# SrinivasBaskar1995/DistributedVolunteerComputing

Hardware: AMD Instinct MI355X
Metric: samples/sec GPT-2-small local-SGD (higher is better)
Workload: dtype bf16; 1 GPU; model=gpt2, global_batch=64, per_peer_batch=64, seq_len=1024, parallelism=local-sgd dp1 H=4 allreduce=direct

## Files before the change

distributedvolunteercomputing_amd/config.py:

```python
from __future__ import annotations

import contextlib
import dataclasses
import os
import threading


def _bool(s: str) -> bool:
    return s.strip().lower() in ("1", "true", "yes", "on")


@dataclasses.dataclass
class RuntimeConfig:
    gemm: str = "lib"
    mlp: str = "fused"
    narrow_gemm: str = "lib"
    mlp_grad_fwd: bool = True
    gemm_fwd: str = "lib"
    dgrad_ps: bool = True
    gemm_wgrad: str = "vcx"
    wgrad_wide: bool = True
    wgrad_ragged: bool = False
    gemm_select: bool = False
    wgrad_big_split_min_m: int = 16384
    async_wgrad: bool = False
    lmhead_chunk: int = 0
    force_reference_ops: bool = False
    tunableop: str = "on"
    tunableop_file: str = ""
    offload_arch: str = "gfx950"
    colour_native: bool = True
    register_source: bool = True
# ... 13 lines not shown
    elastic_liveness: bool = True
    elastic_stage_joins: str = "gloo"
    uplink_pipeline: str = "relay"
    shared_source_root: str = ""
    store_port_train: int = 29611
    store_port_video: int = 29612
    trace_dir: str = ""
    metrics_dir: str = ""


_ENV = {
    "gemm": ("VCX_GEMM", str),
    "mlp": ("VCX_MLP", str),
    "dgrad_ps": ("VCX_DGRAD_PS", _bool),
    "mlp_grad_fwd": ("VCX_MLP_GRAD_FWD", _bool),
    "narrow_gemm": ("VCX_NARROW_GEMM", str),
    "resnet_conv1x1": ("VCX_RESNET_CONV1X1", str),
    "resnet_bn": ("VCX_RESNET_BN", str),
    "resnet_join": ("VCX_RESNET_JOIN", _bool),
    "engine_batch": ("VCX_ENGINE_BATCH", int),
    "conv3x3_wgrad": ("VCX_CONV3X3_WGRAD", str),
    "conv3x3_fwd": ("VCX_CONV3X3_FWD", str),
    "resnet_proj_join": ("VCX_RESNET_PROJ_JOIN", _bool),
    "bn_layer_ws": ("VCX_BN_LAYER_WS", _bool),
    "conv_find": ("VCX_CONV_FIND", _bool),
    "gemm_wgrad": ("VCX_GEMM_WGRAD", str),
    "gemm_fwd": ("VCX_GEMM_FWD", str),
    "wgrad_wide": ("VCX_WGRAD_WIDE", _bool),
    "wgrad_ragged": ("VCX_WGRAD_RAGGED", _bool),
    "gemm_select": ("VCX_GEMM_SELECT", _bool),
# ... 83 lines not shown
```

distributedvolunteercomputing_amd/csrc/bindings.cpp:

```cpp
#include <torch/extension.h>
#include <map>
#include <mutex>
#include <thread>
#include <tuple>
#include <c10/hip/HIPStream.h>
#include <hip/hip_runtime.h>

#include "kernels/vcx_api.h"

namespace {

hipStream_t cur_stream() { return c10::hip::getCurrentHIPStream().stream(); }

#define CHECK_CUDA(x) TORCH_CHECK((x).is_cuda(), #x " must be a GPU tensor")
#define CHECK_CONTIG(x) TORCH_CHECK((x).is_contiguous(), #x " must be contiguous")
#define CHECK_DT(x, dt) TORCH_CHECK((x).scalar_type() == (dt), #x " has wrong dtype ", (x).scalar_type())
#define CHECK_IN(x, dt) \
  CHECK_CUDA(x);        \
  CHECK_CONTIG(x);      \
  CHECK_DT(x, dt)

const auto kBF = at::kBFloat16;
const auto kF = at::kFloat;

// ... 487 lines not shown
              "x under 2 GB");
  for (const at::Tensor* t : {&dy, &x, &out})
    TORCH_CHECK(reinterpret_cast<uintptr_t>(t->data_ptr()) % 16 == 0, "gemm_wg_conv3x3: 16-B aligned base pointers");
  at::Tensor ws = at::empty({splits, Cout, 9 * Cin}, dy.options().dtype(at::kFloat));
  vcx_gemm_wg_conv3x3(dy.data_ptr(), x.data_ptr(), ws.data_ptr<float>(), out.data_ptr(), (int)Cout, (int)Cin, (int)imgs,
                      (int)H, (int)W, (int)stride, (int)splits, accumulate ? 1 : 0, cur_stream());
}

at::Tensor transpose_bf16(at::Tensor src, c10::optional<at::Tensor> dst) {
  TORCH_CHECK(src.is_cuda() && src.dim() == 2 && src.is_contiguous() && src.scalar_type() == at::kBFloat16,
              "transpose_bf16: contiguous 2-D bf16");
  at::Tensor out = dst ? *dst : at::empty({src.size(1), src.size(0)}, src.options());
  TORCH_CHECK(out.size(0) == src.size(1) && out.size(1) == src.size(0) && out.is_contiguous(), "transpose_bf16: dst");
  vcx_transpose_bf16(src.data_ptr(), out.data_ptr(), (int)src.size(0), (int)src.size(1), cur_stream());
  return out;
}

void add_f32_into_bf16(at::Tensor in, at::Tensor out, bool accumulate, bool zero_in) {
  TORCH_CHECK(in.is_cuda() && in.scalar_type() == at::kFloat && out.scalar_type() == at::kBFloat16 &&
                  in.numel() == out.numel() && in.is_contiguous() && out.is_contiguous() &&
                  in.get_device() == out.get_device() && in.numel() < (int64_t(1) << 31),
              "add_f32_into_bf16: fp32 in, bf16 out of equal size on one device");
  vcx_add_f32_into_bf16(in.data_ptr<float>(), out.data_ptr(), (int)in.numel(), accumulate ? 1 : 0, zero_in ? 1 : 0,
                        cur_stream());
}

void reduce_bcast_bf16(at::Tensor in, c10::optional<at::Tensor> out, c10::optional<at::Tensor> mine, int64_t P) {
  TORCH_CHECK(in.is_cuda() && in.scalar_type() == at::kBFloat16 && in.is_contiguous(), "reduce_bcast: bf16 cuda in");
  const int64_t n = in.numel() / P;
  TORCH_CHECK(P > 0 && n * P == in.numel() && n % 8 == 0, "reduce_bcast: numel must be P * n with n % 8 == 0");
// ... 503 lines not shown
  m.def("gemm_f_conv3x3", &gemm_f_conv3x3, py::arg("x"), py::arg("w"), py::arg("out"), py::arg("stride"),
        py::arg("bias") = py::none(), py::arg("waves") = 0, py::arg("splits") = -1, py::arg("flip_taps") = false);
  m.def("gemm_f_splits", &gemm_f_splits, py::arg("M"), py::arg("N"), py::arg("K"));
  m.def("gemm_f", &gemm_f, py::arg("a"), py::arg("b"), py::arg("out"), py::arg("bias") = py::none(),
        py::arg("waves") = 0, py::arg("splits") = -1);
  m.def("gemm_wg_supported", &gemm_wg_supported, py::arg("M"), py::arg("N"), py::arg("K"), py::arg("splits") = 0);
  m.def("gemm_wg_conv3x3_supported", &gemm_wg_conv3x3_supported, py::arg("Cout"), py::arg("Cin"), py::arg("imgs"),
        py::arg("H"), py::arg("W"), py::arg("stride"));
  m.def("gemm_wg_conv3x3", &gemm_wg_conv3x3, py::arg("dy"), py::arg("x"), py::arg("out"), py::arg("accumulate") = false,
        py::arg("stride") = 1, py::arg("splits") = 0);
  m.def("gemm_wg", &gemm_wg, py::arg("a"), py::arg("b"), py::arg("out"), py::arg("accumulate") = false,
        py::arg("splits") = 0, py::arg("loaders") = 8);
  m.def("gemm_nt", &gemm_nt, py::arg("a"), py::arg("b"), py::arg("c"), py::arg("c2") = py::none(),
        py::arg("bias") = py::none(), py::arg("colsum") = py::none(), py::arg("epi") = 0);
  m.def("transpose_bf16", &transpose_bf16, py::arg("src"), py::arg("dst") = py::none());
  m.def("subsample_nhwc", &subsample_nhwc, py::arg("x"), py::arg("stride"));
  m.def("subsample_add_nhwc", &subsample_add_nhwc, py::arg("full"), py::arg("g"), py::arg("stride"));
  m.def("bcast_hw_nhwc", &bcast_hw_nhwc, py::arg("g"), py::arg("H"), py::arg("W"), py::arg("scale"));
  m.def("add_f32_into_bf16", &add_f32_into_bf16, py::arg("src"), py::arg("out"), py::arg("accumulate"),
        py::arg("zero_src") = false);
  m.def("splitk_reduce", &splitk_reduce);
  m.def("ln_fwd", &ln_fwd);
  m.def("ln_bwd", &ln_bwd, pybind11::arg("dy"), pybind11::arg("x"), pybind11::arg("w"), pybind11::arg("mean"),
        pybind11::arg("rstd"), pybind11::arg("dres"), pybind11::arg("has_bias"), pybind11::arg("rms"),
        pybind11::arg("has_bb"), pybind11::arg("dw_out") = pybind11::none(), pybind11::arg("db_out") = pybind11::none(),
        pybind11::arg("dbb_out") = pybind11::none());
  m.def("colsum_bf16", &colsum_bf16, pybind11::arg("y"), pybind11::arg("out") = pybind11::none());
  m.def("gelu_fwd", &gelu_fwd);
  m.def("bias_gelu_fwd", &bias_gelu_fwd);
  m.def("bias_gelu_bwd", &bias_gelu_bwd, pybind11::arg("x"), pybind11::arg("b"), pybind11::arg("dy"),
// ... 27 lines not shown
```

distributedvolunteercomputing_amd/csrc/kernels/gemm.hip:

```cpp
#include <type_traits>

#include "lds_ring.h"

namespace vcx {
namespace gemm {

constexpr int BM = 256, BN = 256, BKS = 32, NSLOT = 4, NT = 512;
constexpr int ROWB = BKS * 2;
constexpr int SLOT_A = BM * ROWB;
constexpr int SLOT_BYTES = (BM + BN) * ROWB;
constexpr int LDS_BYTES = NSLOT * SLOT_BYTES;

enum Epi { EPI_STORE = 0, EPI_BIAS = 1, EPI_BIAS_GELU = 2, EPI_DGELU = 3, EPI_BIAS_RELU = 4 };

__device__ __forceinline__ void glds16(const bf16* g, char* lds) {
  __builtin_amdgcn_global_load_lds((const __attribute__((address_space(1))) void*)g,
                                   (__attribute__((address_space(3))) void*)lds, 16, 0, 0);
}

__device__ __forceinline__ float gelu_tanh(float x) {
  const float u2 = 1.5957691216057308f * fmaf(0.044715f * x, x * x, x);
  return x / (1.f + __expf(-u2));
}

// ... 211 lines not shown
  if constexpr (EPI == EPI_DGELU) {
#pragma unroll
    for (int j = 0; j < 4; ++j)
#pragma unroll
      for (int t = 0; t < 4; ++t) {
        float v = cs[j][t];
        v += __shfl_xor(v, 1, 64);
        v += __shfl_xor(v, 2, 64);
        v += __shfl_xor(v, 4, 64);
        v += __shfl_xor(v, 8, 64);
        if ((lane & 15) == 0) atomicAdd(colsum + ncol + 16 * j + t, v);
      }
  }
}

__global__ void __launch_bounds__(256) transpose_bf16_kernel(const bf16* __restrict__ src, bf16* __restrict__ dst,
                                                             int R, int Cc) {
  __shared__ bf16 t[64][65];
  const int r0 = blockIdx.y * 64, c0 = blockIdx.x * 64;
  for (int e = threadIdx.x; e < 64 * 64; e += 256) {
    const int rr = e >> 6, cc = e & 63;
    if (r0 + rr < R && c0 + cc < Cc) t[rr][cc] = src[(int64_t)(r0 + rr) * Cc + c0 + cc];
  }
  __syncthreads();
  for (int e = threadIdx.x; e < 64 * 64; e += 256) {
    const int cc = e >> 6, rr = e & 63;
    if (r0 + rr < R && c0 + cc < Cc) dst[(int64_t)(c0 + cc) * R + r0 + rr] = t[rr][cc];
  }
}

__global__ void __launch_bounds__(256) transpose_bf16_v8_kernel(const bf16* __restrict__ src, bf16* __restrict__ dst,
                                                                int R, int Cc) {
  __shared__ __attribute__((aligned(16))) bf16 t[64][72];
  const int r0 = blockIdx.y * 64, c0 = blockIdx.x * 64;
#pragma unroll
  for (int i = 0; i < 2; ++i) {
    const int e = threadIdx.x + 256 * i, rr = e >> 3, cc = (e & 7) * 8;
    if (r0 + rr < R && c0 + cc < Cc) *(bf16x8*)&t[rr][cc] = *(const bf16x8*)(src + (int64_t)(r0 + rr) * Cc + c0 + cc);
  }
  __syncthreads();
#pragma unroll
  for (int i = 0; i < 2; ++i) {
    const int e = threadIdx.x + 256 * i, cc = e >> 3, rr = (e & 7) * 8;
    if (c0 + cc < Cc && r0 + rr < R) {
      bf16x8 v;
#pragma unroll
      for (int j = 0; j < 8; ++j) v[j] = t[rr + j][cc];
      *(bf16x8*)(dst + (int64_t)(c0 + cc) * R + r0 + rr) = v;
    }
  }
}

__global__ void __launch_bounds__(256) add_f32_into_bf16_kernel(float* __restrict__ in, bf16* __restrict__ out, int n,
                                                                int accumulate, int zero_in) {
  const int i = blockIdx.x * 256 + threadIdx.x;
  if (i < n) {
    out[i] = (bf16)((accumulate ? (float)out[i] : 0.f) + in[i]);
    if (zero_in) in[i] = 0.f;
  }
}

}
}

using namespace vcx;
// ... 31 lines not shown
    case EPI_BIAS_RELU: args(gemm_nt_kernel<EPI_BIAS_RELU>); break;
    default: args(gemm_nt_kernel<EPI_DGELU>); break;
  }
}

void vcx_transpose_bf16(const void* src, void* dst, int R, int Cc, hipStream_t s) {
  if (R % 8 == 0 && Cc % 8 == 0 && ((uintptr_t)src | (uintptr_t)dst) % 16 == 0) {
    hipLaunchKernelGGL(gemm::transpose_bf16_v8_kernel, dim3((Cc + 63) / 64, (R + 63) / 64), dim3(256), 0, s,
                       (const bf16*)src, (bf16*)dst, R, Cc);
    return;
  }
  hipLaunchKernelGGL(gemm::transpose_bf16_kernel, dim3((Cc + 63) / 64, (R + 63) / 64), dim3(256), 0, s,
                     (const bf16*)src, (bf16*)dst, R, Cc);
}

void vcx_add_f32_into_bf16(float* in, void* out, int n, int accumulate, int zero_in, hipStream_t s) {
  hipLaunchKernelGGL(gemm::add_f32_into_bf16_kernel, dim3((n + 255) / 256), dim3(256), 0, s, in, (bf16*)out, n,
                     accumulate, zero_in);
}
```

distributedvolunteercomputing_amd/csrc/kernels/vcx_api.h:

```cpp
#pragma once
#include <hip/hip_runtime.h>
#include <stdint.h>

void vcx_grad_sumsq(const void* g, int64_t n, float* ostate, hipStream_t s);
void vcx_adam_prologue(float* ostate, float max_norm, hipStream_t s);
void vcx_adamw_flat(void* param, const void* grad, float* master, float* m, float* v, int64_t n, int64_t n_decay,
                    const float* ostate, float beta1, float beta2, float eps, float wd, hipStream_t s);
void vcx_adamw_flat_compact(void* param, const void* grad, float* master, uint8_t* m_code, uint8_t* m_exp,
                            void* v_half, uint8_t* v_exp, int64_t n, int64_t n_decay, const float* ostate,
                            double beta1, double beta2, float eps, float wd, hipStream_t s);
void vcx_optstate_encode(const float* m, const float* v, uint8_t* m_code, uint8_t* m_exp, void* v_half,
                         uint8_t* v_exp, int64_t n, hipStream_t s);
void vcx_optstate_decode(const uint8_t* m_code, const uint8_t* m_exp, const void* v_half, const uint8_t* v_exp,
                         float* m, float* v, int64_t n, hipStream_t s);
void vcx_lsgd_delta(const float* master, const float* anchor, void* delta, int64_t n, hipStream_t s);
void vcx_lsgd_apply(const void* avg, float* anchor, float* master, void* param, float* mom, int64_t n,
                    float outer_lr, float mu, int nesterov, float avg_scale, hipStream_t s);
void vcx_f32_to_bf16(const float* src, void* dst, int64_t n, hipStream_t s);
void vcx_axpy_bf16(const void* src, void* acc, int64_t n, float scale, hipStream_t s);
bool vcx_gemm_wg_supported(int M, int N, int K, int splits);
int vcx_gemm_wg_splits(int M, int N, int K);
void vcx_gemm_wg(const void* A, const void* B, float* Cpart, void* out, int M, int N, int K, int lda, int ldb,
                 int splits, int accumulate, int loaders, hipStream_t s);
bool vcx_gemm_wg_conv3x3_supported(int Cout, int Cin, int tokens, int64_t xbytes, int splits);
// ... 5 lines not shown
void vcx_gemm_f(const void* A, const void* B, void* C, const void* bias, int M, int N, int K, int lda, int ldb,
                int ldc, int waves, int splits, float* ws, hipStream_t s);
bool vcx_gemm_f_conv3x3_supported(int imgs, int H, int W, int Cin, int Cout, int stride);
void vcx_gemm_f_conv3x3(const void* x, const void* w, void* y, const void* bias, int imgs, int H, int W, int Cin,
                        int Cout, int stride, int waves, int splits, float* ws, int flip, int tap_major,
                        hipStream_t s);
bool vcx_gemm_nt_supported(int M, int N, int K);
bool vcx_gemm_nt_supported_epi(int M, int N, int K, int epi);
void vcx_gemm_nt(const void* A, const void* B, void* C, void* C2, const void* bias, float* colsum, int M, int N, int K,
                 int lda, int ldb, int ldc, int epi, hipStream_t s);
bool vcx_gemm_ps_supported(int M, int N, int K, int epi);
int vcx_gemm_ps_grid(int M, int N, int grid_cap);
void vcx_gemm_ps(const void* A, const void* B, void* C, void* C2, const void* bias, float* colsum, int M, int N,
                 int K, int lda, int ldb, int ldc, int epi, int grid_cap, hipStream_t s);
void vcx_transpose_bf16(const void* src, void* dst, int R, int Cc, hipStream_t s);
void vcx_add_f32_into_bf16(float* in, void* out, int n, int accumulate, int zero_in, hipStream_t s);
void vcx_reduce_bcast_bf16(const void* in, void* out, void* mine, int P, int64_t n, hipStream_t s);
void vcx_splitk_reduce(const void* part, void* acc, int S, int64_t n, int accumulate, hipStream_t s);

void vcx_trimmed_reduce_bcast_bf16(const void* in, void* out, void* mine, int P, int64_t n, int trim,
                                   uint32_t live_mask, float inv, int64_t* counts, hipStream_t s);
void vcx_cclip_reduce_bcast_bf16(const void* in, void* out, void* mine, int P, int64_t n, uint32_t live_mask, float tau,
                                 int iters, float* weights, float* workspace, hipStream_t s);
int64_t vcx_cclip_workspace_floats(int P, int64_t n);
int vcx_cclip_max_workgroups();

void vcx_ln_fwd(const void* a, const void* b, void* xout, void* y, const void* w, const void* bias, float* mean,
                float* rstd, int R, int C, float eps, int rms, const void* bb, hipStream_t s);
int vcx_bias_gelu_partials(int R);
void vcx_bias_gelu_fwd(const void* x, const void* b, void* y, int R, int F, hipStream_t s);
// ... 58 lines not shown
```

distributedvolunteercomputing_amd/models/gpt2.py:

```python
from __future__ import annotations

import math
from dataclasses import dataclass

import torch
import torch.nn as nn
import torch.nn.functional as F
from torch.nn.attention import SDPBackend, sdpa_kernel

from .. import ops

_SDPA_BACKENDS = [SDPBackend.EFFICIENT_ATTENTION, SDPBackend.FLASH_ATTENTION, SDPBackend.MATH]


@dataclass
class GPT2Config:
    vocab_size: int = 50257
    padded_vocab: int = 50304
    n_ctx: int = 1024
    n_layer: int = 12
    n_head: int = 12
    n_embd: int = 768
    ln_eps: float = 1e-5

    @staticmethod
# ... 15 lines not shown
        C = cfg.n_embd
        self.n_head = cfg.n_head
        self.ln1_w = nn.Parameter(torch.ones(C))
        self.ln1_b = nn.Parameter(torch.zeros(C))
        self.attn_w = nn.Parameter(torch.empty(3 * C, C))
        self.attn_b = nn.Parameter(torch.zeros(3 * C))
        self.proj_w = nn.Parameter(torch.empty(C, C))
        self.proj_b = nn.Parameter(torch.zeros(C))
        self.ln2_w = nn.Parameter(torch.ones(C))
        self.ln2_b = nn.Parameter(torch.zeros(C))
        self.fc_w = nn.Parameter(torch.empty(4 * C, C))
        self.fc_b = nn.Parameter(torch.zeros(4 * C))
        self.fc2_w = nn.Parameter(torch.empty(C, 4 * C))
        self.fc2_b = nn.Parameter(torch.zeros(C))

    def attn(self, h):
        B, T, C = h.shape
        H = self.n_head
        fuse = (C // H == 64 and h.dtype == torch.bfloat16 and ops.native_linear_ok(self.attn_w)
                and self.attn_b.requires_grad)
        qkv = ops.linear(h, self.attn_w, self.attn_b, bias_grad_elsewhere=fuse).view(B, T, 3, H, C // H)
        if C // H == 64 and qkv.is_cuda:
            y = ops.causal_attention(qkv, bias=self.attn_b if fuse else None)
        else:
            q, k, v = qkv.permute(2, 0, 3, 1, 4).unbind(0)
            with sdpa_kernel(_SDPA_BACKENDS):
                y = F.scaled_dot_product_attention(q, k, v, is_causal=True)
            y = y.transpose(1, 2)
        return ops.linear(y.reshape(B, T, C), self.proj_w)

    def mlp(self, h):
        return ops.mlp_gelu(h, self.fc_w, self.fc_b, self.fc2_w)


class GPT2(nn.Module):
    def __init__(self, cfg: GPT2Config):
        super().__init__()
        self.cfg = cfg
        C = cfg.n_embd
        self.wte = nn.Parameter(torch.empty(cfg.padded_vocab, C))
        self.wpe = nn.Parameter(torch.empty(cfg.n_ctx, C))
        self.blocks = nn.ModuleList([Block(cfg) for _ in range(cfg.n_layer)])
        self.lnf_w = nn.Parameter(torch.ones(C))
        self.lnf_b = nn.Parameter(torch.zeros(C))
        self.reset_parameters()

    @torch.no_grad()
    def reset_parameters(self, seed: int | None = None):
        g = torch.Generator(device="cpu")
        g.manual_seed(1234 if seed is None else seed)
        std = 0.02
        proj_std = 0.02 / math.sqrt(2 * self.cfg.n_layer)

        def init(p, s):
            p.copy_(torch.randn(p.shape, generator=g) * s)

        init(self.wte, std)
        init(self.wpe, 0.01)
        for b in self.blocks:
# ... 1 lines not shown
            init(b.proj_w, proj_std)
            init(b.fc_w, std)
            init(b.fc2_w, proj_std)

    def num_params(self, non_embedding=True):
        n = sum(p.numel() for p in self.parameters())
        if non_embedding:
            n -= self.wpe.numel()
        return n

    def flops_per_token(self, T: int) -> float:
        c = self.cfg
        N = self.num_params(non_embedding=True)
        return 6.0 * N + 12.0 * c.n_layer * c.n_embd * T

    def forward(self, idx, targets=None):
        B, T = idx.shape
        cfg = self.cfg
        x = ops.embed(idx, self.wte, self.wpe)
        eps = cfg.ln_eps
        blocks = self.blocks
        h, resid = ops.add_layernorm(x, None, blocks[0].ln1_w, blocks[0].ln1_b, eps)
        for i, blk in enumerate(blocks):
            a = blk.attn(h)
            h, resid = ops.add_layernorm(resid, a, blk.ln2_w, blk.ln2_b, eps, branch_bias=blk.proj_b)
            m = blk.mlp(h)
            if i + 1 < len(blocks):
                nxt = blocks[i + 1]
                h, resid = ops.add_layernorm(resid, m, nxt.ln1_w, nxt.ln1_b, eps, branch_bias=blk.fc2_b)
            else:
                h, resid = ops.add_layernorm(resid, m, self.lnf_w, self.lnf_b, eps, branch_bias=blk.fc2_b)
        if targets is None:
            return ops.linear(h, self.wte)[..., : cfg.vocab_size]
        return ops.lm_head_cross_entropy(h, self.wte, targets, cfg.vocab_size)
```

distributedvolunteercomputing_amd/ops/__init__.py:

```python
from ._lib import available as native_available, native
from .activations import bias_gelu, gelu, swiglu
from .attention import causal_attention, fused_bias_grad_ok, gqa_attention
from .embedding import embed
from .linear import gemm_nt, linear, mlp_gelu, native_linear_ok, set_gemm_backend, wgrad
from .loss import cross_entropy, lm_head_cross_entropy
from .norm import add_layernorm, add_rmsnorm, layernorm, rmsnorm
from .rope import rope_qkv
from .optim import (CompactState, adamw_flat_compact, adamw_step, adamw_step_compact, axpy_bf16,
                    check_compact_betas, f32_to_bf16, lsgd_apply, lsgd_delta, new_ostate, reduce_bcast_bf16)
from .robust import (centered_clip_reference, cclip_reduce_bcast_bf16, trimmed_mean_reference,
                     trimmed_reduce_bcast_bf16)
```

distributedvolunteercomputing_amd/ops/linear.py:

```python
from __future__ import annotations

import torch
import torch.nn.functional as F


from .. import config
from ._lib import grad_buffer, native, use_native

MIN_ROWS_PER_SPLIT = 2048


def set_gemm_backend(name: str):
    config.update(gemm="lib" if name == "lib" else "vcx")


def gemm_nt_ok(M: int, N: int, K: int, t) -> bool:
    return (config.get().gemm == "vcx" and use_native(t) and t.dtype == torch.bfloat16
            and bool(native().gemm_nt_supported(M, N, K)))


def gemm_nt(a, b, bias=None, out=None):
    a = a if a.stride(-1) == 1 else a.contiguous()
    out = torch.empty(a.shape[0], b.shape[0], device=a.device, dtype=a.dtype) if out is None else out
    native().gemm_nt(a, b, out, None, bias, None, 1 if bias is not None else 0)
# ... 18 lines not shown


def gemm_f_ok(M: int, N: int, K: int, t) -> bool:
    return (config.get().gemm_fwd == "vcx" and use_native(t) and t.dtype == torch.bfloat16 and t.is_contiguous()
            and bool(native().gemm_f_supported(M, N, K)))


def gemm_f(a, w, bias=None):
    out = torch.empty(a.shape[0], w.shape[0], device=a.device, dtype=a.dtype)
    native().gemm_f(a, w.contiguous(), out, bias)
    return out


def transpose_weight(w):
    return native().transpose_bf16(w.contiguous())
_CHOICE: dict = {}


def _torch_mm(a, b, trans_a, trans_b, bias):
    if trans_b and not trans_a:
        return F.linear(a, b, bias)
    y = torch.mm(a.t() if trans_a else a, b.t() if trans_b else b)
    return y if bias is None else y.add_(bias)


def _lt_mm(a, b, trans_a, trans_b, bias):
    C = native()
    M = a.shape[1] if trans_a else a.shape[0]
    N = b.shape[0] if trans_b else b.shape[1]
    out = torch.empty(M, N, device=a.device, dtype=a.dtype)
# ... 202 lines not shown
            full[:, ::s, ::s, :] = g
        return full.permute(0, 3, 1, 2), None, None


def _nhwc_hip_ok(t: torch.Tensor) -> bool:
    return (use_native(t) and t.dtype == torch.bfloat16 and t.dim() == 4 and t.is_contiguous() and t.shape[3] % 8 == 0
            and t.data_ptr() % 16 == 0)


def subsample_tap(x: torch.Tensor, join: GradJoin, stride: int) -> torch.Tensor:
    return _SubsampleTap.apply(x, join, stride)


class _Linear(torch.autograd.Function):
    @staticmethod
    def forward(ctx, x, w, b, bias_grad_elsewhere=False, join=None, deposit=False):
        ctx.save_for_backward(x, w)
        ctx.has_bias = b is not None and not bias_grad_elsewhere
        ctx.bias = b
        ctx.join, ctx.deposit = join, deposit
        if deposit:
            join.pending, join.ran = None, False
        x2 = x.reshape(-1, x.shape[-1])
        w = _w2(w)
        if gemm_nt_ok(x2.shape[0], w.shape[0], x2.shape[1], x2):
            return gemm_nt(x2, w, b).view(*x.shape[:-1], w.shape[0])
        if gemm_f_ok(x2.shape[0], w.shape[0], x2.shape[1], x2) and (b is None or b.is_contiguous()):
            return gemm_f(x2, w, b).view(*x.shape[:-1], w.shape[0])
        if b is None and narrow_gemm_ok(x2.shape[0], w.shape[0], x2.shape[1], x2):
            return narrow_gemm(x2, w).view(*x.shape[:-1], w.shape[0])
        return mm(x2, w, trans_b=True, bias=b).view(*x.shape[:-1], w.shape[0])

    @staticmethod
    def backward(ctx, dy):
        x, w_param = ctx.saved_tensors
# ... 3 lines not shown
        x2 = x.reshape(-1, K)
        dy2 = dy2.contiguous()
        dx = None
        join, ctx.join = ctx.join, None
        deposit = ctx.deposit
        if deposit:
            join, depo = None, join
        base = join.take() if join is not None else None
        if join is not None and base is None:
            join.ran = True
        if ctx.needs_input_grad[0] and base is not None and base.shape == (dy2.shape[0], K) and base.is_contiguous():
            dx = base.addmm_(dy2, w).view(x.shape)
        elif base is not None:
            dx = (mm(dy2, w) + base).view(x.shape) if ctx.needs_input_grad[0] else None
        elif ctx.needs_input_grad[0]:
            if gemm_nt_ok(dy2.shape[0], K, N, dy2):
                dx = gemm_nt(dy2, transpose_weight(w)).view(x.shape)
            elif gemm_f_ok(dy2.shape[0], K, N, dy2):
                dx = gemm_f(dy2, transpose_weight(w)).view(x.shape)
            elif narrow_gemm_ok(dy2.shape[0], K, N, dy2):
                dx = narrow_gemm(dy2, transpose_weight(w)).view(x.shape)
            elif dgrad_ps_ok(dy2.shape[0], K, N, dy2):
                dx = torch.empty(dy2.shape[0], K, device=dy2.device, dtype=dy2.dtype)
                native().gemm_ps(dy2, transpose_weight(w), dx)
                dx = dx.view(x.shape)
            else:
                dx = mm(dy2, w).view(x.shape)
        if deposit and dx is not None and not depo.ran and dx.is_contiguous():
            depo.pending, dx = dx.view(-1, K), None
        want_w = bool(ctx.needs_input_grad[1])
        want_b = bool(ctx.has_bias and ctx.needs_input_grad[2])
        bias, ctx.bias = ctx.bias, None
        w = w_param
        flat_w = w.grad is not None and w.grad.is_contiguous() and w.grad.dtype == w.dtype
        flat_b = (not want_b) or grad_buffer(bias) is not None
        if config.get().async_wgrad and dy2.is_cuda and flat_w and flat_b and (want_w or want_b):
            main = torch.cuda.current_stream(dy2.device)
            side = _side_stream(dy2.device)
            side.wait_stream(main)
            with torch.cuda.stream(side):
                _param_grads(dy2, x2, w, bias, want_w, want_b)
            dy2.record_stream(side)
            x2.record_stream(side)
            _queue_join(main, side, dy2.device)
            return dx, None, None, None, None, None
        dw, db = _param_grads(dy2, x2, w, bias, want_w, want_b)
        return dx, dw, db, None, None, None


def native_linear_ok(w: torch.Tensor) -> bool:
    return use_native(w) and w.dtype == torch.bfloat16 and torch.is_grad_enabled() and w.requires_grad


def linear(x: torch.Tensor, w: torch.Tensor, b: torch.Tensor | None = None,
           bias_grad_elsewhere: bool = False, join: GradJoin | None = None, deposit: bool = False) -> torch.Tensor:
    if native_linear_ok(w):
        return _Linear.apply(x, w, b, bias_grad_elsewhere, join, deposit)
    assert join is None, "a GradJoin needs the native linear path (its backward consumes the joined gradient)"
    return F.linear(x, _w2(w), b)


def dgrad_ps_ok(M: int, N: int, K: int, t) -> bool:
    return (config.get().dgrad_ps and K <= 2304 and use_native(t) and t.dtype == torch.bfloat16
            and t.is_contiguous() and bool(native().gemm_ps_supported(M, N, K, 0)))


def gemm_ps_ok(M: int, N: int, K: int, epi: int, t) -> bool:
    return (config.get().mlp == "fused" and use_native(t) and t.dtype == torch.bfloat16
            and bool(native().gemm_ps_supported(M, N, K, epi)))


class _MlpGelu(torch.autograd.Function):

    @staticmethod
    def forward(ctx, x, w1, b1, w2, ps):
        C = native()
        x2 = x.reshape(-1, x.shape[-1])
        M, F_ = x2.shape[0], w1.shape[0]
        pre = torch.empty(M, F_, device=x.device, dtype=x.dtype)
        act = torch.empty_like(pre)
        if ps:
            C.gemm_ps(x2, w1, pre, act, b1, None, 5 if config.get().mlp_grad_fwd else 2)
            y = gemm_f(act, w2) if gemm_f_ok(M, w2.shape[0], F_, act) else mm(act, w2, trans_b=True)
        else:
            C.gemm_nt(x2, w1, pre, act, b1, None, 2)
            y = gemm_nt(act, w2)
        ctx.save_for_backward(x2, w1, b1, w2, pre, act)
        ctx.xshape = x.shape
        ctx.ps = ps
        ctx.grad_fwd = bool(ps and config.get().mlp_grad_fwd)
        return y.view(*x.shape[:-1], w2.shape[0])

    @staticmethod
    def backward(ctx, dy):
        C = native()
        x2, w1, b1, w2, pre, act = ctx.saved_tensors
        dy2 = dy.reshape(-1, dy.shape[-1]).contiguous()
        M, F_ = pre.shape
        gb = grad_buffer(b1) if ctx.needs_input_grad[2] else None
        cs = _colsum_buffer(F_, dy.device) if gb is not None else torch.zeros(F_, device=dy.device, dtype=torch.float32)
        dpre = torch.empty_like(pre)
        if ctx.ps:
            C.gemm_ps(dy2, transpose_weight(w2), dpre, pre, None, cs, 6 if ctx.grad_fwd else 4)
        else:
            C.gemm_nt(dy2, transpose_weight(w2), dpre, pre, None, cs, 3)
        dw2, _ = _param_grads(dy2, act, w2, None, ctx.needs_input_grad[3], False)
        dw1, _ = _param_grads(dpre, x2, w1, None, ctx.needs_input_grad[1], False)
        db1 = None
        if ctx.needs_input_grad[2]:
            if gb is not None:
                C.add_f32_into_bf16(cs, gb, True, True)
            else:
                db1 = cs.to(b1.dtype)
        dx = None
        if ctx.needs_input_grad[0]:
            dx = (mm(dpre, w1) if ctx.ps else gemm_nt(dpre, transpose_weight(w1))).view(ctx.xshape)
        return dx, dw1, db1, dw2, None


_COLSUM = {}


def _colsum_buffer(n: int, device) -> torch.Tensor:
    key = (n, device, torch.cuda.current_stream(device).cuda_stream)
    buf = _COLSUM.get(key)
    if buf is None:
        buf = _COLSUM[key] = torch.zeros(n, device=device, dtype=torch.float32)
    return buf


def mlp_gelu_ok(x, w1, w2) -> bool:
    return _mlp_mode(x, w1, w2) is not None


def _mlp_mode(x, w1, w2):
    if not (native_linear_ok(w1) and x.dtype == torch.bfloat16):
        return None
    M = x.numel() // x.shape[-1]
    F_, C_ = w1.shape
    if gemm_ps_ok(M, F_, C_, 2, x) and gemm_ps_ok(M, F_, w2.shape[0], 4, x):
        return "ps"
    if (gemm_nt_ok(M, F_, C_, x) and gemm_nt_ok(M, w2.shape[0], F_, x) and gemm_nt_ok(M, C_, w2.shape[0], x)
            and gemm_nt_ok(M, F_, w2.shape[0], x)):
        return "nt"
    return None


def mlp_gelu(x, w1, b1, w2):
    mode = _mlp_mode(x, w1, w2)
    if mode is not None:
        return _MlpGelu.apply(x, w1, b1, w2, mode == "ps")
    from .activations import bias_gelu

    return linear(bias_gelu(linear(x, w1), b1), w2)
```

distributedvolunteercomputing_amd/ops/loss.py:

```python
from __future__ import annotations

import torch
import torch.nn.functional as F

from .. import config
from ._lib import native, use_native


class _XEntFused(torch.autograd.Function):
    @staticmethod
    def forward(ctx, logits, targets, vocab, ignore_index, nvalid, loss_rows):
        ctx.logits = logits
        return loss_rows.sum() / nvalid

    @staticmethod
    def backward(ctx, dloss):
        d = ctx.logits
        ctx.logits = None
        native().xent_rescale(d, dloss.float().reshape(1).contiguous())
        return d, None, None, None, None, None


class _XEnt(torch.autograd.Function):
    @staticmethod
# ... 66 lines not shown

    @staticmethod
    def backward(ctx, dloss):
        from .linear import _param_grads, mm

        x2, w = ctx.saved_tensors
        d, ctx.d = ctx.d, None
        native().xent_rescale(d, dloss.float().reshape(1).contiguous())
        dx = mm(d, w) if ctx.needs_input_grad[0] else None
        dw = None
        if ctx.needs_input_grad[1]:
            dw, _ = _param_grads(d, x2, w, None, True, False)
        return dx, dw, None, None, None, None


def lm_head_cross_entropy(x, w, targets, vocab: int, chunk: int | None = None):
    from .linear import linear

    x2 = x.reshape(-1, x.shape[-1])
    t = targets.reshape(-1)
    mc = config.get().lmhead_chunk if chunk is None else chunk
    Vp = w.shape[0]
    if (mc and use_native(x2) and torch.is_grad_enabled() and x2.dtype == torch.bfloat16 and Vp % 8 == 0
            and Vp <= 57344 and x2.shape[0] > mc):
        t = t.contiguous().long()
        nvalid = (t >= 0).sum().clamp_min(1).to(torch.float32).reshape(1)
        return _LMHeadXEnt.apply(x2.contiguous(), w, t, vocab, nvalid, mc)
    return cross_entropy(linear(x2, w), t, vocab=vocab)
```

Baseline: 1099 samples/s.

## Batch all weight transposes into one grouped kernel launch at forward start

```diff
diff --git a/distributedvolunteercomputing_amd/config.py b/distributedvolunteercomputing_amd/config.py
--- a/distributedvolunteercomputing_amd/config.py
+++ b/distributedvolunteercomputing_amd/config.py
@@ -16,6 +16,9 @@
     mlp: str = "fused"
     narrow_gemm: str = "lib"
     mlp_grad_fwd: bool = True
+    bwd_batch: bool = True
+    fc_dgrad_nt: bool = True
+    lmhead_dgrad_nt: bool = True
     gemm_fwd: str = "lib"
     dgrad_ps: bool = True
     gemm_wgrad: str = "vcx"
@@ -59,6 +62,9 @@
     "mlp": ("VCX_MLP", str),
     "dgrad_ps": ("VCX_DGRAD_PS", _bool),
     "mlp_grad_fwd": ("VCX_MLP_GRAD_FWD", _bool),
+    "bwd_batch": ("VCX_BWD_BATCH", _bool),
+    "fc_dgrad_nt": ("VCX_FC_DGRAD_NT", _bool),
+    "lmhead_dgrad_nt": ("VCX_LMHEAD_DGRAD_NT", _bool),
     "narrow_gemm": ("VCX_NARROW_GEMM", str),
     "resnet_conv1x1": ("VCX_RESNET_CONV1X1", str),
     "resnet_bn": ("VCX_RESNET_BN", str),
diff --git a/distributedvolunteercomputing_amd/csrc/bindings.cpp b/distributedvolunteercomputing_amd/csrc/bindings.cpp
--- a/distributedvolunteercomputing_amd/csrc/bindings.cpp
+++ b/distributedvolunteercomputing_amd/csrc/bindings.cpp
@@ -525,6 +525,38 @@
   TORCH_CHECK(out.size(0) == src.size(1) && out.size(1) == src.size(0) && out.is_contiguous(), "transpose_bf16: dst");
   vcx_transpose_bf16(src.data_ptr(), out.data_ptr(), (int)src.size(0), (int)src.size(1), cur_stream());
   return out;
+}
+
+std::tuple<std::vector<at::Tensor>, int64_t> transpose_bf16_many(std::vector<at::Tensor> srcs,
+                                                                 c10::optional<std::vector<at::Tensor>> dsts) {
+  TORCH_CHECK(!dsts || dsts->size() == srcs.size(), "transpose_bf16_many: one dst per src");
+  std::vector<at::Tensor> outs;
+  std::vector<vcx::TransposeJob> jobs;
+  outs.reserve(srcs.size());
+  jobs.reserve(srcs.size());
+  for (size_t i = 0; i < srcs.size(); ++i) {
+    const at::Tensor& src = srcs[i];
+    TORCH_CHECK(src.is_cuda() && src.dim() == 2 && src.is_contiguous() && src.scalar_type() == at::kBFloat16 &&
+                    src.get_device() == srcs[0].get_device() && src.size(0) <= INT32_MAX && src.size(1) <= INT32_MAX,
+                "transpose_bf16_many: contiguous 2-D bf16 on one device");
+    at::Tensor out = dsts ? (*dsts)[i] : at::empty({src.size(1), src.size(0)}, src.options());
+    TORCH_CHECK(out.dim() == 2 && out.size(0) == src.size(1) && out.size(1) == src.size(0) && out.is_contiguous() &&
+                    out.scalar_type() == at::kBFloat16 && out.is_cuda() && out.get_device() == src.get_device(),
+                "transpose_bf16_many: dst");
+    vcx::TransposeJob j{};
+    j.src = src.data_ptr();
+    j.dst = out.data_ptr();
+    j.R = (int)src.size(0);
+    j.Cc = (int)src.size(1);
+    jobs.push_back(j);
+    outs.push_back(std::move(out));
+  }
+  int launches = 0;
+  if (!jobs.empty()) {
+    launches = vcx_transpose_bf16_many(jobs.data(), (int)jobs.size(), cur_stream());
+    TORCH_CHECK(launches >= 0, "transpose_bf16_many: a matrix of more than 2^31 tiles");
+  }
+  return {std::move(outs), (int64_t)launches};
 }
 
 void add_f32_into_bf16(at::Tensor in, at::Tensor out, bool accumulate, bool zero_in) {
@@ -1058,6 +1090,8 @@
   m.def("gemm_nt", &gemm_nt, py::arg("a"), py::arg("b"), py::arg("c"), py::arg("c2") = py::none(),
         py::arg("bias") = py::none(), py::arg("colsum") = py::none(), py::arg("epi") = 0);
   m.def("transpose_bf16", &transpose_bf16, py::arg("src"), py::arg("dst") = py::none());
+  m.def("transpose_bf16_many", &transpose_bf16_many, py::arg("srcs"), py::arg("dsts") = py::none());
+  m.attr("JOB_TABLE_CAP") = (int64_t)vcx::JOBS_MAX;
   m.def("subsample_nhwc", &subsample_nhwc, py::arg("x"), py::arg("stride"));
   m.def("subsample_add_nhwc", &subsample_add_nhwc, py::arg("full"), py::arg("g"), py::arg("stride"));
   m.def("bcast_hw_nhwc", &bcast_hw_nhwc, py::arg("g"), py::arg("H"), py::arg("W"), py::arg("scale"));
diff --git a/distributedvolunteercomputing_amd/csrc/kernels/gemm.hip b/distributedvolunteercomputing_amd/csrc/kernels/gemm.hip
--- a/distributedvolunteercomputing_amd/csrc/kernels/gemm.hip
+++ b/distributedvolunteercomputing_amd/csrc/kernels/gemm.hip
@@ -1,5 +1,6 @@
 #include <type_traits>
 
+#include "job_table.h"
 #include "lds_ring.h"
 
 namespace vcx {
@@ -249,10 +250,8 @@
   }
 }
 
-__global__ void __launch_bounds__(256) transpose_bf16_kernel(const bf16* __restrict__ src, bf16* __restrict__ dst,
-                                                             int R, int Cc) {
-  __shared__ bf16 t[64][65];
-  const int r0 = blockIdx.y * 64, c0 = blockIdx.x * 64;
+__device__ __forceinline__ void transpose_tile(const bf16* __restrict__ src, bf16* __restrict__ dst, int R, int Cc,
+                                               int r0, int c0, bf16 (*t)[65]) {
   for (int e = threadIdx.x; e < 64 * 64; e += 256) {
     const int rr = e >> 6, cc = e & 63;
     if (r0 + rr < R && c0 + cc < Cc) t[rr][cc] = src[(int64_t)(r0 + rr) * Cc + c0 + cc];
@@ -264,10 +263,8 @@
   }
 }
 
-__global__ void __launch_bounds__(256) transpose_bf16_v8_kernel(const bf16* __restrict__ src, bf16* __restrict__ dst,
-                                                                int R, int Cc) {
-  __shared__ __attribute__((aligned(16))) bf16 t[64][72];
-  const int r0 = blockIdx.y * 64, c0 = blockIdx.x * 64;
+__device__ __forceinline__ void transpose_tile_v8(const bf16* __restrict__ src, bf16* __restrict__ dst, int R, int Cc,
+                                                  int r0, int c0, bf16 (*t)[72]) {
 #pragma unroll
   for (int i = 0; i < 2; ++i) {
     const int e = threadIdx.x + 256 * i, rr = e >> 3, cc = (e & 7) * 8;
@@ -284,6 +281,33 @@
       *(bf16x8*)(dst + (int64_t)(c0 + cc) * R + r0 + rr) = v;
     }
   }
+}
+
+__global__ void __launch_bounds__(256) transpose_bf16_kernel(const bf16* __restrict__ src, bf16* __restrict__ dst,
+                                                             int R, int Cc) {
+  __shared__ bf16 t[64][65];
+  transpose_tile(src, dst, R, Cc, blockIdx.y * 64, blockIdx.x * 64, t);
+}
+
+__global__ void __launch_bounds__(256) transpose_bf16_v8_kernel(const bf16* __restrict__ src, bf16* __restrict__ dst,
+                                                                int R, int Cc) {
+  __shared__ __attribute__((aligned(16))) bf16 t[64][72];
+  transpose_tile_v8(src, dst, R, Cc, blockIdx.y * 64, blockIdx.x * 64, t);
+}
+
+__global__ void __launch_bounds__(256) transpose_bf16_many_kernel(const TransposeTable tab) {
+  __shared__ __attribute__((aligned(16))) bf16 t[64 * 72];
+  const int b = blockIdx.x;
+  const int j = job_of_workgroup(tab.first, tab.njobs, b);
+  const int tile = b - tab.first[j], tx = tab.job[j].tiles_x;
+  const int r0 = (tile / tx) * 64, c0 = (tile % tx) * 64;
+  const bf16* src = (const bf16*)tab.job[j].src;
+  bf16* dst = (bf16*)tab.job[j].dst;
+  const int R = tab.job[j].R, Cc = tab.job[j].Cc;
+  if (tab.job[j].v8)
+    transpose_tile_v8(src, dst, R, Cc, r0, c0, (bf16(*)[72])t);
+  else
+    transpose_tile(src, dst, R, Cc, r0, c0, (bf16(*)[65])t);
 }
 
 __global__ void __launch_bounds__(256) add_f32_into_bf16_kernel(float* __restrict__ in, bf16* __restrict__ out, int n,
@@ -345,6 +369,19 @@
                      (const bf16*)src, (bf16*)dst, R, Cc);
 }
 
+int vcx_transpose_bf16_many(const vcx::TransposeJob* jobs, int n, hipStream_t s) {
+  int launches = 0;
+  for (int i = 0; i < n;) {
+    TransposeTable tab{};
+    i = pack_transpose_jobs(jobs, n, i, &tab);
+    if (i < 0) return -1;
+    if (tab.njobs == 0) break;
+    hipLaunchKernelGGL(gemm::transpose_bf16_many_kernel, dim3(tab.first[tab.njobs]), dim3(256), 0, s, tab);
+    ++launches;
+  }
+  return launches;
+}
+
 void vcx_add_f32_into_bf16(float* in, void* out, int n, int accumulate, int zero_in, hipStream_t s) {
   hipLaunchKernelGGL(gemm::add_f32_into_bf16_kernel, dim3((n + 255) / 256), dim3(256), 0, s, in, (bf16*)out, n,
                      accumulate, zero_in);
diff --git a/distributedvolunteercomputing_amd/csrc/kernels/job_table.h b/distributedvolunteercomputing_amd/csrc/kernels/job_table.h
--- /dev/null
+++ b/distributedvolunteercomputing_amd/csrc/kernels/job_table.h
@@ -0,0 +1,54 @@
+#pragma once
+#include <stdint.h>
+
+namespace vcx {
+
+constexpr int JOBS_MAX = 64;
+
+struct TransposeJob {
+  const void* src;
+  void* dst;
+  int R, Cc;
+  int tiles_x;
+  int v8;
+};
+
+struct TransposeTable {
+  int njobs;
+  int first[JOBS_MAX + 1];
+  TransposeJob job[JOBS_MAX];
+};
+
+inline int pack_transpose_jobs(const TransposeJob* jobs, int n, int start, TransposeTable* t) {
+  t->njobs = 0;
+  t->first[0] = 0;
+  int i = start < 0 ? 0 : start;
+  for (; i < n && t->njobs < JOBS_MAX; ++i) {
+    const TransposeJob& in = jobs[i];
+    if (in.R <= 0 || in.Cc <= 0) continue;
+    const int64_t tx = ((int64_t)in.Cc + 63) / 64, ty = ((int64_t)in.R + 63) / 64;
+    if (tx * ty > INT32_MAX) return -1;
+    const int64_t end = (int64_t)t->first[t->njobs] + tx * ty;
+    if (end > INT32_MAX) break;
+    TransposeJob& o = t->job[t->njobs];
+    o = in;
+    o.tiles_x = (int)tx;
+    o.v8 = (in.R % 8 == 0 && in.Cc % 8 == 0 && ((uintptr_t)in.src | (uintptr_t)in.dst) % 16 == 0) ? 1 : 0;
+    t->first[++t->njobs] = (int)end;
+  }
+  return i;
+}
+
+#if defined(__HIPCC__)
+__host__ __device__
+#endif
+inline int job_of_workgroup(const int* first, int njobs, int b) {
+  int lo = 0, hi = njobs;
+  while (hi - lo > 1) {
+    const int mid = (lo + hi) >> 1;
+    if (first[mid] <= b) lo = mid; else hi = mid;
+  }
+  return lo;
+}
+
+}
diff --git a/distributedvolunteercomputing_amd/csrc/kernels/vcx_api.h b/distributedvolunteercomputing_amd/csrc/kernels/vcx_api.h
--- a/distributedvolunteercomputing_amd/csrc/kernels/vcx_api.h
+++ b/distributedvolunteercomputing_amd/csrc/kernels/vcx_api.h
@@ -1,6 +1,8 @@
 #pragma once
 #include <hip/hip_runtime.h>
 #include <stdint.h>
+
+#include "job_table.h"
 
 void vcx_grad_sumsq(const void* g, int64_t n, float* ostate, hipStream_t s);
 void vcx_adam_prologue(float* ostate, float max_norm, hipStream_t s);
@@ -43,6 +45,7 @@
 void vcx_gemm_ps(const void* A, const void* B, void* C, void* C2, const void* bias, float* colsum, int M, int N,
                  int K, int lda, int ldb, int ldc, int epi, int grid_cap, hipStream_t s);
 void vcx_transpose_bf16(const void* src, void* dst, int R, int Cc, hipStream_t s);
+int vcx_transpose_bf16_many(const vcx::TransposeJob* jobs, int n, hipStream_t s);
 void vcx_add_f32_into_bf16(float* in, void* out, int n, int accumulate, int zero_in, hipStream_t s);
 void vcx_reduce_bcast_bf16(const void* in, void* out, void* mine, int P, int64_t n, hipStream_t s);
 void vcx_splitk_reduce(const void* part, void* acc, int S, int64_t n, int accumulate, hipStream_t s);
diff --git a/distributedvolunteercomputing_amd/models/gpt2.py b/distributedvolunteercomputing_amd/models/gpt2.py
--- a/distributedvolunteercomputing_amd/models/gpt2.py
+++ b/distributedvolunteercomputing_amd/models/gpt2.py
@@ -8,7 +8,7 @@
 import torch.nn.functional as F
 from torch.nn.attention import SDPBackend, sdpa_kernel
 
-from .. import ops
+from .. import config, ops
 
 _SDPA_BACKENDS = [SDPBackend.EFFICIENT_ATTENTION, SDPBackend.FLASH_ATTENTION, SDPBackend.MATH]
 
@@ -54,12 +54,12 @@
         self.fc2_w = nn.Parameter(torch.empty(C, 4 * C))
         self.fc2_b = nn.Parameter(torch.zeros(C))
 
-    def attn(self, h):
+    def attn(self, h, attn_wt=None, proj_wt=None):
         B, T, C = h.shape
         H = self.n_head
         fuse = (C // H == 64 and h.dtype == torch.bfloat16 and ops.native_linear_ok(self.attn_w)
                 and self.attn_b.requires_grad)
-        qkv = ops.linear(h, self.attn_w, self.attn_b, bias_grad_elsewhere=fuse).view(B, T, 3, H, C // H)
+        qkv = ops.linear(h, self.attn_w, self.attn_b, bias_grad_elsewhere=fuse, wt=attn_wt).view(B, T, 3, H, C // H)
         if C // H == 64 and qkv.is_cuda:
             y = ops.causal_attention(qkv, bias=self.attn_b if fuse else None)
         else:
@@ -67,10 +67,10 @@
             with sdpa_kernel(_SDPA_BACKENDS):
                 y = F.scaled_dot_product_attention(q, k, v, is_causal=True)
             y = y.transpose(1, 2)
-        return ops.linear(y.reshape(B, T, C), self.proj_w)
+        return ops.linear(y.reshape(B, T, C), self.proj_w, wt=proj_wt)
 
-    def mlp(self, h):
-        return ops.mlp_gelu(h, self.fc_w, self.fc_b, self.fc2_w)
+    def mlp(self, h, fc_wt=None, fc2_wt=None):
+        return ops.mlp_gelu(h, self.fc_w, self.fc_b, self.fc2_w, w1t=fc_wt, w2t=fc2_wt)
 
 
 class GPT2(nn.Module):
@@ -83,6 +83,7 @@
         self.blocks = nn.ModuleList([Block(cfg) for _ in range(cfg.n_layer)])
         self.lnf_w = nn.Parameter(torch.ones(C))
         self.lnf_b = nn.Parameter(torch.zeros(C))
+        self._wt_bufs = None
         self.reset_parameters()
 
     @torch.no_grad()
@@ -114,6 +115,24 @@
         N = self.num_params(non_embedding=True)
         return 6.0 * N + 12.0 * c.n_layer * c.n_embd * T
 
+    def _weight_transposes(self, h, chunked_head=False):
+        blocks = self.blocks
+        b0 = blocks[0]
+        none = [(None, None, None, None)] * len(blocks), None
+        if not (config.get().bwd_batch and torch.is_grad_enabled() and h.dtype == torch.bfloat16
+                and ops.native_linear_ok(b0.attn_w)):
+            return none
+        M = h.numel() // h.shape[-1]
+        want = (ops.linear_wants_wt(M, b0.attn_w, h), ops.linear_wants_wt(M, b0.proj_w, h),
+                *ops.mlp_wants_wt(h, b0.fc_w, b0.fc2_w))
+        want_lm = not chunked_head and (ops.linear_wants_wt(M, self.wte, h) or config.get().lmhead_dgrad_nt)
+        if not (any(want) or want_lm):
+            return none
+        ws = [w for b in blocks for w, use in zip((b.attn_w, b.proj_w, b.fc_w, b.fc2_w), want) if use]
+        self._wt_bufs = ops.transpose_weights(ws + ([self.wte] if want_lm else []), self._wt_bufs)
+        it = iter(self._wt_bufs)
+        return [tuple(next(it) if use else None for use in want) for _ in blocks], (next(it) if want_lm else None)
+
     def forward(self, idx, targets=None):
         B, T = idx.shape
         cfg = self.cfg
@@ -121,15 +140,18 @@
         eps = cfg.ln_eps
         blocks = self.blocks
         h, resid = ops.add_layernorm(x, None, blocks[0].ln1_w, blocks[0].ln1_b, eps)
+        mc = config.get().lmhead_chunk
+        wts, wte_t = self._weight_transposes(h, chunked_head=targets is not None and bool(mc) and B * T > mc)
         for i, blk in enumerate(blocks):
-            a = blk.attn(h)
+            attn_wt, proj_wt, fc_wt, fc2_wt = wts[i]
+            a = blk.attn(h, attn_wt, proj_wt)
             h, resid = ops.add_layernorm(resid, a, blk.ln2_w, blk.ln2_b, eps, branch_bias=blk.proj_b)
-            m = blk.mlp(h)
+            m = blk.mlp(h, fc_wt, fc2_wt)
             if i + 1 < len(blocks):
                 nxt = blocks[i + 1]
                 h, resid = ops.add_layernorm(resid, m, nxt.ln1_w, nxt.ln1_b, eps, branch_bias=blk.fc2_b)
             else:
                 h, resid = ops.add_layernorm(resid, m, self.lnf_w, self.lnf_b, eps, branch_bias=blk.fc2_b)
         if targets is None:
-            return ops.linear(h, self.wte)[..., : cfg.vocab_size]
-        return ops.lm_head_cross_entropy(h, self.wte, targets, cfg.vocab_size)
+            return ops.linear(h, self.wte, wt=wte_t)[..., : cfg.vocab_size]
+        return ops.lm_head_cross_entropy(h, self.wte, targets, cfg.vocab_size, wt=wte_t)
diff --git a/distributedvolunteercomputing_amd/ops/__init__.py b/distributedvolunteercomputing_amd/ops/__init__.py
--- a/distributedvolunteercomputing_amd/ops/__init__.py
+++ b/distributedvolunteercomputing_amd/ops/__init__.py
@@ -3,6 +3,7 @@
 from .attention import causal_attention, fused_bias_grad_ok, gqa_attention
 from .embedding import embed
 from .linear import gemm_nt, linear, mlp_gelu, native_linear_ok, set_gemm_backend, wgrad
+from .linear import linear_wants_wt, mlp_wants_wt, transpose_weights
 from .loss import cross_entropy, lm_head_cross_entropy
 from .norm import add_layernorm, add_rmsnorm, layernorm, rmsnorm
 from .rope import rope_qkv
diff --git a/distributedvolunteercomputing_amd/ops/linear.py b/distributedvolunteercomputing_amd/ops/linear.py
--- a/distributedvolunteercomputing_amd/ops/linear.py
+++ b/distributedvolunteercomputing_amd/ops/linear.py
@@ -56,6 +56,29 @@
 
 def transpose_weight(w):
     return native().transpose_bf16(w.contiguous())
+
+
+def transpose_weights(ws, out=None):
+    ws = [w.contiguous() for w in ws]
+    if out is not None and not (len(out) == len(ws) and all(
+            o.shape == (w.shape[1], w.shape[0]) and o.device == w.device and o.dtype == w.dtype for o, w in zip(out, ws))):
+        out = None
+    return native().transpose_bf16_many(ws, out)[0]
+
+
+def linear_wants_wt(M: int, w, t) -> bool:
+    N, K = _w2(w).shape
+    return (gemm_nt_ok(M, K, N, t) or gemm_f_ok(M, K, N, t) or narrow_gemm_ok(M, K, N, t) or dgrad_ps_ok(M, K, N, t))
+
+
+def mlp_wants_wt(x, w1, w2):
+    mode = _mlp_mode(x, w1, w2)
+    if mode is None:
+        M = x.numel() // x.shape[-1]
+        return linear_wants_wt(M, w1, x), linear_wants_wt(M, w2, x)
+    return mode == "nt" or bool(config.get().fc_dgrad_nt), True
+
+
 _CHOICE: dict = {}
 
 
@@ -288,11 +311,12 @@
 
 class _Linear(torch.autograd.Function):
     @staticmethod
-    def forward(ctx, x, w, b, bias_grad_elsewhere=False, join=None, deposit=False):
+    def forward(ctx, x, w, b, bias_grad_elsewhere=False, join=None, deposit=False, wt=None):
         ctx.save_for_backward(x, w)
         ctx.has_bias = b is not None and not bias_grad_elsewhere
         ctx.bias = b
         ctx.join, ctx.deposit = join, deposit
+        ctx.wt = wt
         if deposit:
             join.pending, join.ran = None, False
         x2 = x.reshape(-1, x.shape[-1])
@@ -326,16 +350,19 @@
         elif base is not None:
             dx = (mm(dy2, w) + base).view(x.shape) if ctx.needs_input_grad[0] else None
         elif ctx.needs_input_grad[0]:
+            wt = ctx.wt
             if gemm_nt_ok(dy2.shape[0], K, N, dy2):
-                dx = gemm_nt(dy2, transpose_weight(w)).view(x.shape)
+                dx = gemm_nt(dy2, transpose_weight(w) if wt is None else wt).view(x.shape)
             elif gemm_f_ok(dy2.shape[0], K, N, dy2):
-                dx = gemm_f(dy2, transpose_weight(w)).view(x.shape)
+                dx = gemm_f(dy2, transpose_weight(w) if wt is None else wt).view(x.shape)
             elif narrow_gemm_ok(dy2.shape[0], K, N, dy2):
-                dx = narrow_gemm(dy2, transpose_weight(w)).view(x.shape)
+                dx = narrow_gemm(dy2, transpose_weight(w) if wt is None else wt).view(x.shape)
             elif dgrad_ps_ok(dy2.shape[0], K, N, dy2):
                 dx = torch.empty(dy2.shape[0], K, device=dy2.device, dtype=dy2.dtype)
-                native().gemm_ps(dy2, transpose_weight(w), dx)
+                native().gemm_ps(dy2, transpose_weight(w) if wt is None else wt, dx)
                 dx = dx.view(x.shape)
+            elif wt is not None:
+                dx = mm(dy2, wt, trans_b=True).view(x.shape)
             else:
                 dx = mm(dy2, w).view(x.shape)
         if deposit and dx is not None and not depo.ran and dx.is_contiguous():
@@ -355,9 +382,9 @@
             dy2.record_stream(side)
             x2.record_stream(side)
             _queue_join(main, side, dy2.device)
-            return dx, None, None, None, None, None
+            return dx, None, None, None, None, None, None
         dw, db = _param_grads(dy2, x2, w, bias, want_w, want_b)
-        return dx, dw, db, None, None, None
+        return dx, dw, db, None, None, None, None
 
 
 def native_linear_ok(w: torch.Tensor) -> bool:
@@ -365,9 +392,10 @@
 
 
 def linear(x: torch.Tensor, w: torch.Tensor, b: torch.Tensor | None = None,
-           bias_grad_elsewhere: bool = False, join: GradJoin | None = None, deposit: bool = False) -> torch.Tensor:
+           bias_grad_elsewhere: bool = False, join: GradJoin | None = None, deposit: bool = False,
+           wt: torch.Tensor | None = None) -> torch.Tensor:
     if native_linear_ok(w):
-        return _Linear.apply(x, w, b, bias_grad_elsewhere, join, deposit)
+        return _Linear.apply(x, w, b, bias_grad_elsewhere, join, deposit, wt)
     assert join is None, "a GradJoin needs the native linear path (its backward consumes the joined gradient)"
     return F.linear(x, _w2(w), b)
 
@@ -385,7 +413,7 @@
 class _MlpGelu(torch.autograd.Function):
 
     @staticmethod
-    def forward(ctx, x, w1, b1, w2, ps):
+    def forward(ctx, x, w1, b1, w2, ps, w1t=None, w2t=None):
         C = native()
         x2 = x.reshape(-1, x.shape[-1])
         M, F_ = x2.shape[0], w1.shape[0]
@@ -400,6 +428,7 @@
         ctx.save_for_backward(x2, w1, b1, w2, pre, act)
         ctx.xshape = x.shape
         ctx.ps = ps
+        ctx.w1t, ctx.w2t = w1t, w2t
         ctx.grad_fwd = bool(ps and config.get().mlp_grad_fwd)
         return y.view(*x.shape[:-1], w2.shape[0])
 
@@ -412,10 +441,12 @@
         gb = grad_buffer(b1) if ctx.needs_input_grad[2] else None
         cs = _colsum_buffer(F_, dy.device) if gb is not None else torch.zeros(F_, device=dy.device, dtype=torch.float32)
         dpre = torch.empty_like(pre)
+        w1t = ctx.w1t
+        w2t = transpose_weight(w2) if ctx.w2t is None else ctx.w2t
         if ctx.ps:
-            C.gemm_ps(dy2, transpose_weight(w2), dpre, pre, None, cs, 6 if ctx.grad_fwd else 4)
+            C.gemm_ps(dy2, w2t, dpre, pre, None, cs, 6 if ctx.grad_fwd else 4)
         else:
-            C.gemm_nt(dy2, transpose_weight(w2), dpre, pre, None, cs, 3)
+            C.gemm_nt(dy2, w2t, dpre, pre, None, cs, 3)
         dw2, _ = _param_grads(dy2, act, w2, None, ctx.needs_input_grad[3], False)
         dw1, _ = _param_grads(dpre, x2, w1, None, ctx.needs_input_grad[1], False)
         db1 = None
@@ -426,8 +457,14 @@
                 db1 = cs.to(b1.dtype)
         dx = None
         if ctx.needs_input_grad[0]:
-            dx = (mm(dpre, w1) if ctx.ps else gemm_nt(dpre, transpose_weight(w1))).view(ctx.xshape)
-        return dx, dw1, db1, dw2, None
+            if not ctx.ps:
+                dx = gemm_nt(dpre, transpose_weight(w1) if w1t is None else w1t)
+            elif w1t is not None and config.get().fc_dgrad_nt:
+                dx = mm(dpre, w1t, trans_b=True)
+            else:
+                dx = mm(dpre, w1)
+            dx = dx.view(ctx.xshape)
+        return dx, dw1, db1, dw2, None, None, None
 
 
 _COLSUM = {}
@@ -458,10 +495,10 @@
     return None
 
 
-def mlp_gelu(x, w1, b1, w2):
+def mlp_gelu(x, w1, b1, w2, w1t=None, w2t=None):
     mode = _mlp_mode(x, w1, w2)
     if mode is not None:
-        return _MlpGelu.apply(x, w1, b1, w2, mode == "ps")
+        return _MlpGelu.apply(x, w1, b1, w2, mode == "ps", w1t, w2t)
     from .activations import bias_gelu
 
-    return linear(bias_gelu(linear(x, w1), b1), w2)
+    return linear(bias_gelu(linear(x, w1, wt=w1t), b1), w2, wt=w2t)
diff --git a/distributedvolunteercomputing_amd/ops/loss.py b/distributedvolunteercomputing_amd/ops/loss.py
--- a/distributedvolunteercomputing_amd/ops/loss.py
+++ b/distributedvolunteercomputing_amd/ops/loss.py
@@ -104,7 +104,7 @@
         return dx, dw, None, None, None, None
 
 
-def lm_head_cross_entropy(x, w, targets, vocab: int, chunk: int | None = None):
+def lm_head_cross_entropy(x, w, targets, vocab: int, chunk: int | None = None, wt=None):
     from .linear import linear
 
     x2 = x.reshape(-1, x.shape[-1])
@@ -116,4 +116,4 @@
         t = t.contiguous().long()
         nvalid = (t >= 0).sum().clamp_min(1).to(torch.float32).reshape(1)
         return _LMHeadXEnt.apply(x2.contiguous(), w, t, vocab, nvalid, mc)
-    return cross_entropy(linear(x2, w), t, vocab=vocab)
+    return cross_entropy(linear(x2, w, wt=wt), t, vocab=vocab)
```

Measured after the change: 1113 samples/s (median of 6 runs). 1.01x the previous value.
